# LeCAR-Lab/CoVO-MPC

Hardware: AMD Instinct MI355X
Metric: mpc_control_steps_per_sec (higher is better)
Workload: dtype f32; 1 GPU; covo-online tracking_zigzag N=65536 H=32 lam=0.01 sigma=0.5 (teacher-forced on the recorded inputs -- noisy state, a_mean, key -- of this controller's own 300-step closed-loop episode, timed steps spread evenly over the episode; samples sharded 1x65536, one exchange of the 516-float rank records per step: collective); controller=covo-online, task=tracking_zigzag, N_global=65536, N_local=65536, H=32, pos_stats_info=False

## Files before the change

covo_mpc_amd/csrc/hessian_adj_body.hpp:

```cpp
constexpr int NX = ADJ_NX, NZ = NX + 4, NH = NX + 1, HH = COVO_H, NA = COVO_NA;
constexpr size_t WS_X = 0;
constexpr size_t WS_JF = WS_X + 32 * 16;
constexpr size_t WS_GL = WS_JF + 32 * NX * NZ;
constexpr size_t WS_LAM = WS_GL + 32 * 16;
constexpr size_t WS_MXX = WS_LAM + 33 * 16;
constexpr size_t WS_MXU = WS_MXX + 32 * 256;
constexpr size_t WS_MUU = WS_MXU + 32 * 64;
constexpr size_t WS_S = WS_MUU + 32 * 16;
constexpr int NPAIR = NZ * (NZ + 1) / 2;
constexpr int PAIR_THREADS = (NPAIR + 63) / 64 * 64;
constexpr size_t WS_COUNT = WS_S + (size_t)32 * 16 * NA + 2;
constexpr unsigned long long ADJ_LAM_UNSET = 0xFFF7ADEADBEEF000ull;


__device__ __forceinline__ void adj_force(const float *__restrict__ st, const AdjArgs &A, int bi, int k, double (&f)[3])
{
    if (k == 0) {
        f[0] = st[ST_FDIST + 0]; f[1] = st[ST_FDIST + 1]; f[2] = st[ST_FDIST + 2];
    } else if (A.f_tab != nullptr) {
        const float4 r = A.f_tab[(size_t)bi * HH + k];
        f[0] = r.x; f[1] = r.y; f[2] = r.z;
    } else {
        f[0] = f[1] = f[2] = 0.0;
    }
}

__device__ __forceinline__ void adj_targets(const float *__restrict__ st, const float *__restrict__ pos_traj,
                                            const float *__restrict__ vel_traj, int T, int time0, int k, double (&tar)[6])
{
    if (k == 0) {
        for (int i = 0; i < 3; ++i) { tar[i] = st[ST_POSTAR + i]; tar[3 + i] = st[ST_VELTAR + i]; }
    } else {
        int idx = time0 + k;
        idx = idx < 0 ? 0 : (idx > T - 1 ? T - 1 : idx);
        for (int i = 0; i < 3; ++i) { tar[i] = pos_traj[3 * idx + i]; tar[3 + i] = vel_traj[3 * idx + i]; }
    }
}

#define ADJ_FOR_STATE(OP) OP(px, 0) OP(py, 1) OP(pz, 2) OP(vx, 3) OP(vy, 4) OP(vz, 5) OP(qx, 6) OP(qy, 7) OP(qz, 8) OP(qw, 9) OP(ox, 10) OP(oy, 11) OP(oz, 12)

__device__ __forceinline__ void adj_store_state(const qm::State<double> &p, double *__restrict__ x)
{
#define OP(m, i) x[i] = p.m;
    ADJ_FOR_STATE(OP)
#undef OP
}
__device__ __forceinline__ void adj_load_state(qm::State<double> &p, const double *__restrict__ x)
{
#define OP(m, i) p.m = x[i];
    ADJ_FOR_STATE(OP)
#undef OP
}

#if ADJ_FS
struct AdjDrag {
    double k, off[3];
};
__device__ __forceinline__ AdjDrag adj_drag(const AdjArgs &A, int bi)
{
    AdjDrag D = {A.drag_k, {A.drag_off[0], A.drag_off[1], A.drag_off[2]}};
    if (A.models != nullptr) {
        const dm::Model m = A.models[bi];
        D.k = adj_drag_coeff(m);
        for (int i = 0; i < 3; ++i) D.off[i] = 0.5 * (double)m.dp[i];
    }
    return D;
}
template <class S>
__device__ __forceinline__ void adj_next_force(const AdjArgs &A, const AdjDrag &D, int bi, int k, const qm::State<S> &s, const S (&f)[3],
                                               S (&fn)[3])
{
    if (k + 1 >= HH) {
        fn[0] = fn[1] = fn[2] = S{};
        return;
    }
    const float4 r = A.f_tab[(size_t)bi * HH + k + 1];
    const double g[3] = {r.x, r.y, r.z}, c = r.w;
    const S v[3] = {s.vx, s.vy, s.vz};
#pragma unroll
    for (int i = 0; i < 3; ++i) fn[i] = (f[i] * c + g[i]) + qm::drag_force<S, double>(v[i], D.off[i], D.k);
}
#endif


#if !ADJ_FS
struct AdjQuat {
    double x, y, z, w;
};
__device__ __forceinline__ AdjQuat adj_qmul(const AdjQuat &a, const AdjQuat &b)
{
    AdjQuat r;
    r.x = fma(a.w, b.x, fma(a.x, b.w, fma(a.y, b.z, -(a.z * b.y))));
    r.y = fma(a.w, b.y, fma(a.y, b.w, fma(a.z, b.x, -(a.x * b.z))));
    r.z = fma(a.w, b.z, fma(a.z, b.w, fma(a.x, b.y, -(a.y * b.x))));
    r.w = fma(a.w, b.w, -fma(a.x, b.x, fma(a.y, b.y, a.z * b.z)));
    return r;
}
template <int CTRL>
__device__ __forceinline__ AdjQuat adj_qdpp(const AdjQuat &q)
{
    return AdjQuat{wr::dpp_f64<CTRL>(q.x), wr::dpp_f64<CTRL>(q.y), wr::dpp_f64<CTRL>(q.z), wr::dpp_f64<CTRL>(q.w)};
}
__device__ __forceinline__ double adj_scan_sum(double v, const double (&pw)[4], double pr, int lane)
{
    v = fma(wr::dpp_f64<0x111>(v), pw[0], v);
    v = fma(wr::dpp_f64<0x112>(v), pw[1], v);
    v = fma(wr::dpp_f64<0x114>(v), pw[2], v);
    v = fma(wr::dpp_f64<0x118>(v), pw[3], v);
    const double t = wr::dpp_f64<0x142>(v);
    return ((lane & 16) != 0) ? fma(t, pr, v) : v;
}
template <bool FT>
__device__ __forceinline__ qm::State<double> adj_prefix_scan(const qm::State<double> &p0, const double (*sact)[4], const double (*sfd)[3],
                                                             const qm::Consts<double> &c, int lane)
{
    const int k = lane & 31, lo = lane & 15;
    const double one[4] = {1.0, 1.0, 1.0, 1.0};
    double pa[4];
    pa[0] = c.alpha;
    pa[1] = pa[0] * pa[0];
    pa[2] = pa[1] * pa[1];
    pa[3] = pa[2] * pa[2];
    const double a16 = pa[3] * pa[3];
    double alo = 1.0;
    if (lo & 1) alo *= pa[0];
    if (lo & 2) alo *= pa[1];
    if (lo & 4) alo *= pa[2];
    if (lo & 8) alo *= pa[3];
    const double ak = (k & 16) ? alo * a16 : alo, apr = alo * c.alpha;
    const double th = sact[k][0];
    double cx = sact[k][1] * c.one_m_alpha, cy = sact[k][2] * c.one_m_alpha, cz = sact[k][3] * c.one_m_alpha;
    cx = adj_scan_sum(cx, pa, apr, lane);
    cy = adj_scan_sum(cy, pa, apr, lane);
    cz = adj_scan_sum(cz, pa, apr, lane);
    const double ox = fma(ak, p0.ox, wr::dpp_f64<0x138>(cx));
    const double oy = fma(ak, p0.oy, wr::dpp_f64<0x138>(cy));
    const double oz = fma(ak, p0.oz, wr::dpp_f64<0x138>(cz));
    AdjQuat P{ox * c.half_dt, oy * c.half_dt, oz * c.half_dt, 1.0};
    {
        AdjQuat t = adj_qdpp<0x111>(P);
        if (lo >= 1) P = adj_qmul(t, P);
        t = adj_qdpp<0x112>(P);
        if (lo >= 2) P = adj_qmul(t, P);
        t = adj_qdpp<0x114>(P);
        if (lo >= 4) P = adj_qmul(t, P);
        t = adj_qdpp<0x118>(P);
        if (lo >= 8) P = adj_qmul(t, P);
        t = adj_qdpp<0x142>(P);
        if (lane & 16) P = adj_qmul(t, P);
    }
    AdjQuat E = adj_qdpp<0x138>(P);
    if (lane == 0) E = AdjQuat{0.0, 0.0, 0.0, 1.0};
    AdjQuat q0{p0.qx, p0.qy, p0.qz, p0.qw};
    {
        const double rn = qm::rsq64_(fma(q0.x, q0.x, fma(q0.y, q0.y, fma(q0.z, q0.z, q0.w * q0.w))));
        q0.x *= rn; q0.y *= rn; q0.z *= rn; q0.w *= rn;
    }
    AdjQuat q = adj_qmul(q0, E);
    if (k > 0) {
        const double rn = qm::rsq64_(fma(q.x, q.x, fma(q.y, q.y, fma(q.z, q.z, q.w * q.w))));
        q.x *= rn; q.y *= rn; q.z *= rn; q.w *= rn;
    }
    const double fx = (FT || k == 0) ? sfd[k][0] : 0.0, fy = (FT || k == 0) ? sfd[k][1] : 0.0, fz = (FT || k == 0) ? sfd[k][2] : 0.0;
    const double Qz0 = 2.0 * (q.x * q.z + q.y * q.w), Qz1 = 2.0 * (q.y * q.z - q.x * q.w), Qz2 = q.w * q.w - q.x * q.x - q.y * q.y + q.z * q.z;
    double dvx = ((Qz0 * th + fx) * c.inv_m) * c.dt, dvy = ((Qz1 * th + fy) * c.inv_m) * c.dt, dvz = ((Qz2 * th + fz) * c.inv_m + c.neg_g) * c.dt;
    dvx = adj_scan_sum(dvx, one, 1.0, lane);
    dvy = adj_scan_sum(dvy, one, 1.0, lane);
    dvz = adj_scan_sum(dvz, one, 1.0, lane);
    const double vx = p0.vx + wr::dpp_f64<0x138>(dvx), vy = p0.vy + wr::dpp_f64<0x138>(dvy), vz = p0.vz + wr::dpp_f64<0x138>(dvz);
    double dpx = adj_scan_sum(vx * c.dt, one, 1.0, lane), dpy = adj_scan_sum(vy * c.dt, one, 1.0, lane), dpz = adj_scan_sum(vz * c.dt, one, 1.0, lane);
    qm::State<double> r;
    r.px = p0.px + wr::dpp_f64<0x138>(dpx);
    r.py = p0.py + wr::dpp_f64<0x138>(dpy);
    r.pz = p0.pz + wr::dpp_f64<0x138>(dpz);
    r.vx = vx; r.vy = vy; r.vz = vz;
    r.qx = (k == 0) ? p0.qx : q.x; r.qy = (k == 0) ? p0.qy : q.y; r.qz = (k == 0) ? p0.qz : q.z; r.qw = (k == 0) ? p0.qw : q.w;
    r.ox = ox; r.oy = oy; r.oz = oz;
    return r;
}
#endif

__device__ __forceinline__ void adj_hd_step(const float *__restrict__ st, const float *__restrict__ am, const AdjArgs &A, int bi,
                                            int time0, int k, const qm::State<double> &p, int a, int b, qm::HD &r,
                                            qm::State<qm::HD> &s
#if ADJ_FS
                                            , const double (&pf)[3], qm::HD (&fn)[3]
#endif
)
{
    const qm::Consts<double> c = A.cs ? A.cs[bi] : A.c;
#define OP(m, i) s.m = qm::HD{p.m, a == i ? 1.0 : 0.0, b == i ? 1.0 : 0.0, 0.0};
    ADJ_FOR_STATE(OP)
#undef OP
#if ADJ_FS
    qm::HD fh[3];
#pragma unroll
    for (int i = 0; i < 3; ++i) {
        fh[i] = qm::HD{pf[i], a == 13 + i ? 1.0 : 0.0, b == 13 + i ? 1.0 : 0.0, 0.0};
        fn[i] = fh[i];
    }
#endif
    r = qm::hd(0.0);
    if (k >= 1) {
        double tar[6];
        adj_targets(st, A.pos_traj + bi * A.traj_stride, A.vel_traj + bi * A.traj_stride, A.T, time0, k, tar);
        r = qm::reward_kind<qm::HD, double>(A.reward, s, tar[0], tar[1], tar[2], tar[3], tar[4], tar[5]);
    }
    if (k <= HH - 2) {
        qm::HD act[4];
#pragma unroll
        for (int d = 0; d < 4; ++d) {
            const qm::HD x{(double)am[4 * k + d], a == NX + d ? 1.0 : 0.0, b == NX + d ? 1.0 : 0.0, 0.0};
            act[d] = qm::clip11_(qm::clip11_(x));
        }
#if ADJ_FS
        adj_next_force<qm::HD>(A, adj_drag(A, bi), bi, k, s, fh, fn);
        qm::dyn_step<qm::HD, double, true, qm::HD>(s, act[0], act[1], act[2], act[3], c, fh[0], fh[1], fh[2]);
#else
        double f[3];
        adj_force(st, A, bi, k, f);
        qm::dyn_step<qm::HD, double>(s, act[0], act[1], act[2], act[3], c, f[0], f[1], f[2]);
#endif
    }
}

template <bool FT>
__global__ __launch_bounds__(64) void adj_jac_kernel(const AdjArgs A)
{
    const int k = blockIdx.x, b = blockIdx.y, lane = threadIdx.x;
    const float *__restrict__ st = A.state + (size_t)b * COVO_STATE_FLOATS;
    const bool raw = A.a_mean_raw != nullptr;
    const float *__restrict__ am_base = raw ? A.a_mean_raw : A.a_mean + (size_t)b * NA;
    const bool shift = raw && A.begin_pass == 0;
    auto am = [&](int i) { return am_base[(shift && i < NA - 4) ? i + 4 : i]; };
    if (raw && k == 0) {
        float *shift_out = const_cast<float *>(A.a_mean);
        shift_out[lane] = am(lane);
        shift_out[lane + 64] = am(lane + 64);
        if (lane < 4) {
            if (A.begin_pass > 0) {
                const uint32_t p0 = A.dyn_out[10], p1 = A.dyn_out[11];
                uint32_t rk[2];
                step_begin_derive_next(lane, p0, p1, A.shared_noise_scale, A.dyn_out, rk);
            } else {
                step_begin_derive(lane, A.blk, A.derive_keys, A.shared_noise_scale, A.dyn_out);
            }
        }
        if (lane == 4 && A.seq != nullptr) A.seq[0] = A.seq[0] + 1u;
    }
    double *__restrict__ ws = A.ws + (size_t)b * WS_COUNT;
    if (lane < 16) {
        reinterpret_cast<unsigned long long *>(ws + WS_LAM)[16 * k + lane] = ADJ_LAM_UNSET;
        if (k == HH - 1) reinterpret_cast<unsigned long long *>(ws + WS_LAM)[16 * HH + lane] = ADJ_LAM_UNSET;
    }
    const int time0 = __float_as_int(st[ST_TIME]);
    const qm::Consts<double> c = A.cs ? A.cs[b] : A.c;
    qm::State<double> p;
    p.px = st[ST_POS + 0]; p.py = st[ST_POS + 1]; p.pz = st[ST_POS + 2];
    p.vx = st[ST_VEL + 0]; p.vy = st[ST_VEL + 1]; p.vz = st[ST_VEL + 2];
    p.qx = st[ST_QUAT + 0]; p.qy = st[ST_QUAT + 1]; p.qz = st[ST_QUAT + 2]; p.qw = st[ST_QUAT + 3];
    p.ox = st[ST_OMEGA + 0]; p.oy = st[ST_OMEGA + 1]; p.oz = st[ST_OMEGA + 2];
    __shared__ double sact[HH][4];
    __shared__ double sfd[HH][3];
    if (lane < HH) {
        double f[3];
        adj_force(st, A, b, lane, f);
        sfd[lane][0] = f[0]; sfd[lane][1] = f[1]; sfd[lane][2] = f[2];
    }
    if (lane < HH) {
        const double a0 = qm::clip11_((double)am(4 * lane + 0)), a1 = qm::clip11_((double)am(4 * lane + 1));
        const double a2 = qm::clip11_((double)am(4 * lane + 2)), a3 = qm::clip11_((double)am(4 * lane + 3));
        sact[lane][0] = (a0 + 1.0) * c.thrust_half;
        sact[lane][1] = a1 * c.komega[0];
        sact[lane][2] = a2 * c.komega[1];
        sact[lane][3] = a3 * c.komega[2];
    }
    __syncthreads();
#if ADJ_FS
    const AdjDrag D = adj_drag(A, b);
    double pf[3] = {sfd[0][0], sfd[0][1], sfd[0][2]};
    for (int t = 0; t < k; ++t) {
        const double th = sact[t][0], w0 = sact[t][1], w1 = sact[t][2], w2 = sact[t][3];
        double fn[3];
        adj_next_force<double>(A, D, b, t, p, pf, fn);
        if (t == 0) qm::dyn_core<double, double>(p, th, w0, w1, w2, c, pf[0], pf[1], pf[2]);
        else qm::dyn_core<double, double, false>(p, th, w0, w1, w2, c, pf[0], pf[1], pf[2]);
        pf[0] = fn[0]; pf[1] = fn[1]; pf[2] = fn[2];
    }
    if (lane == 0) {
        adj_store_state(p, ws + WS_X + 16 * k);
        ws[WS_X + 16 * k + 13] = pf[0]; ws[WS_X + 16 * k + 14] = pf[1]; ws[WS_X + 16 * k + 15] = pf[2];
    }
#else
    if (A.scan_prefix) {
        const qm::State<double> ps = adj_prefix_scan<FT>(p, sact, sfd, c, lane);
#define OP(m, i) p.m = wr::bcast_lane(ps.m, k);
        ADJ_FOR_STATE(OP)
#undef OP
    } else {
        for (int t = 0; t < k; ++t) {
            const double th = sact[t][0], w0 = sact[t][1], w1 = sact[t][2], w2 = sact[t][3];
            if (t == 0) qm::dyn_core<double, double>(p, th, w0, w1, w2, c, sfd[0][0], sfd[0][1], sfd[0][2]);
            else if (FT) qm::dyn_core<double, double, false>(p, th, w0, w1, w2, c, sfd[t][0], sfd[t][1], sfd[t][2]);
            else qm::dyn_core<double, double, false>(p, th, w0, w1, w2, c, 0.0, 0.0, 0.0);
        }
    }
    if (lane == 0) adj_store_state(p, ws + WS_X + 16 * k);
#endif
    qm::State<qm::D1> s;
#define OP(m, i) s.m = qm::D1{p.m, lane == i ? 1.0 : 0.0};
    ADJ_FOR_STATE(OP)
#undef OP
#if ADJ_FS
    qm::D1 fd[3], fdn[3];
#pragma unroll
    for (int i = 0; i < 3; ++i) {
        fd[i] = qm::D1{pf[i], lane == 13 + i ? 1.0 : 0.0};
        fdn[i] = fd[i];
    }
#endif
    qm::D1 r{0.0, 0.0};
    if (k >= 1) {
        double tar[6];
        adj_targets(st, A.pos_traj + b * A.traj_stride, A.vel_traj + b * A.traj_stride, A.T, time0, k, tar);
        r = qm::reward_kind<qm::D1, double>(A.reward, s, tar[0], tar[1], tar[2], tar[3], tar[4], tar[5]);
    }
    if (k <= HH - 2) {
        qm::D1 act[4];
#pragma unroll
        for (int d = 0; d < 4; ++d) {
            const qm::D1 x{(double)am(4 * k + d), lane == NX + d ? 1.0 : 0.0};
            act[d] = qm::clip11_(qm::clip11_(x));
        }
#if ADJ_FS
        adj_next_force<qm::D1>(A, D, b, k, s, fd, fdn);
        qm::dyn_step<qm::D1, double, true, qm::D1>(s, act[0], act[1], act[2], act[3], c, fd[0], fd[1], fd[2]);
#else
        qm::dyn_step<qm::D1, double>(s, act[0], act[1], act[2], act[3], c, sfd[k][0], sfd[k][1], sfd[k][2]);
#endif
    }
    if (lane < NZ) {
        if (lane < NX) ws[WS_GL + 16 * k + lane] = r.a;
        if (k <= HH - 2) {
            double *__restrict__ jf = ws + WS_JF + (size_t)k * NX * NZ;
#define OP(m, i) jf[i * NZ + lane] = s.m.a;
            ADJ_FOR_STATE(OP)
#undef OP
#if ADJ_FS
            jf[13 * NZ + lane] = fdn[0].a; jf[14 * NZ + lane] = fdn[1].a; jf[15 * NZ + lane] = fdn[2].a;
#endif
        }
    }
}

__device__ __forceinline__ void adj_hd_pairs(const AdjArgs &A, int k, int b, int tid)
{
    if (tid >= NPAIR) return;
    const float *__restrict__ st = A.state + (size_t)b * COVO_STATE_FLOATS;
    const float *__restrict__ am = A.a_mean + (size_t)b * NA;
    double *__restrict__ ws = A.ws + (size_t)b * WS_COUNT;
    const int time0 = __float_as_int(st[ST_TIME]);
    int q = tid, a = 0;
    while (q >= NZ - a) { q -= NZ - a; ++a; }
    const int bb = a + q;
    qm::State<double> p;
    adj_load_state(p, ws + WS_X + 16 * k);
    qm::HD r;
    qm::State<qm::HD> s;
#if ADJ_FS
    const double pf[3] = {ws[WS_X + 16 * k + 13], ws[WS_X + 16 * k + 14], ws[WS_X + 16 * k + 15]};
    qm::HD fn[3];
    adj_hd_step(st, am, A, b, time0, k, p, a, bb, r, s, pf, fn);
#else
    adj_hd_step(st, am, A, b, time0, k, p, a, bb, r, s);
#endif
    double h[NH];
    h[0] = r.ab;
#define OP(m, i) h[1 + i] = s.m.ab;
    ADJ_FOR_STATE(OP)
#undef OP
#if ADJ_FS
    h[14] = fn[0].ab; h[15] = fn[1].ab; h[16] = fn[2].ab;
#endif
    double g = h[0];
    if (k <= HH - 2) {
        const double *__restrict__ Lk = ws + WS_LAM + 16 * (k + 1);
        double lam[NX];
        const long long t0 = wall_clock64();
        for (;;) {
            bool unset = false;
#pragma unroll
            for (int i = 0; i < NX; ++i) {
                lam[i] = __hip_atomic_load(Lk + i, __ATOMIC_RELAXED, __HIP_MEMORY_SCOPE_AGENT);
                unset |= (unsigned long long)__double_as_longlong(lam[i]) == ADJ_LAM_UNSET;
            }
            if (!unset) break;
            if (wall_clock64() - t0 > 50000000LL) {
                if (A.status != nullptr) __hip_atomic_fetch_or(A.status, COVO_DEVSTAT_ADJOINT, __ATOMIC_RELAXED, __HIP_MEMORY_SCOPE_SYSTEM);
                break;
            }
            __builtin_amdgcn_s_sleep(2);
        }
#pragma unroll
        for (int i = 0; i < NX; ++i) g = fma(lam[i], h[1 + i], g);
    }
    double *__restrict__ Mxx = ws + WS_MXX + (size_t)k * 256, *__restrict__ Mxu = ws + WS_MXU + (size_t)k * 64;
    double *__restrict__ Muu = ws + WS_MUU + (size_t)k * 16;
    if (bb < NX) {
        Mxx[a * 16 + bb] = g;
        Mxx[bb * 16 + a] = g;
    } else if (a < NX) {
        Mxu[a * 4 + (bb - NX)] = g;
    } else {
        Muu[(a - NX) * 4 + (bb - NX)] = g;
        Muu[(bb - NX) * 4 + (a - NX)] = g;
    }
}

__device__ __forceinline__ void adj_hd_padding(const AdjArgs &A, int k, int b, int tid, int nthreads)
{
    double *__restrict__ ws = A.ws + (size_t)b * WS_COUNT;
    double *__restrict__ Mxx = ws + WS_MXX + (size_t)k * 256, *__restrict__ Mxu = ws + WS_MXU + (size_t)k * 64;
    for (int e = tid; e < 256; e += nthreads)
        if ((e >> 4) >= NX || (e & 15) >= NX) Mxx[e] = 0.0;
    if (tid < (16 - NX) * 4) Mxu[NX * 4 + tid] = 0.0;
}

__global__ __launch_bounds__(256) void adj_hd_kernel(const AdjArgs A)
{
    adj_hd_padding(A, (int)blockIdx.x, (int)blockIdx.y, (int)threadIdx.x, 256);
    adj_hd_pairs(A, (int)blockIdx.x, (int)blockIdx.y, (int)threadIdx.x);
}

static_assert(HH == 32, "adj_chain_kernel: four horizon segments of 8, 8, 8 and 7 steps");
constexpr int KC_ZI = (HH - 1) * NX * NZ;
constexpr int KC_TLD = 17;

__device__ __forceinline__ void adj_wave_sync()
{
    __builtin_amdgcn_fence(__ATOMIC_ACQ_REL, "wavefront");
    __builtin_amdgcn_wave_barrier();
}
__device__ __forceinline__ void adj_cd_to_a(double *__restrict__ tb, const f64x4 &t, int lo, int hi, double (&a)[4])
{
    adj_wave_sync();
#pragma unroll
    for (int r = 0; r < 4; ++r) tb[(4 * r + hi) * KC_TLD + lo] = t[r];
    adj_wave_sync();
#pragma unroll
    for (int g = 0; g < 4; ++g) a[g] = tb[lo * KC_TLD + 4 * g + hi];
}
__device__ __forceinline__ f64x4 adj_mm(const double (&a)[4], const f64x4 &b, f64x4 acc)
{
#pragma unroll
    for (int g = 0; g < 4; ++g) acc = __builtin_amdgcn_mfma_f64_16x16x4f64(a[g], b[g], acc, 0, 0, 0);
    return acc;
}
template <int CNT>
__device__ __forceinline__ void adj_mm_many(const double (&pa)[8][4], const f64x4 &b, f64x4 (&out)[8])
{
#pragma unroll
    for (int i = 0; i < CNT; ++i) out[i] = f64x4{0.0, 0.0, 0.0, 0.0};
#pragma unroll
    for (int g = 0; g < 4; ++g) {
#pragma unroll
        for (int i = 0; i < CNT; ++i) out[i] = __builtin_amdgcn_mfma_f64_16x16x4f64(pa[i][g], b[g], out[i], 0, 0, 0);
    }
}

template <int J>
__device__ __forceinline__ void adj_sens_chain(const double *__restrict__ sjf, double *__restrict__ tb, double *__restrict__ ho,
                                               double *__restrict__ S, int w, int lane, double (&pa)[8][4], f64x4 &sv)
{
    constexpr int M0 = 8 * J, M1 = J == 3 ? HH - 1 : 8 * J + 8;
    const int lo = lane & 15, hi = lane >> 4;
    const int col = 16 * w + lo, tcol = col >> 2, dcol = col & 3, k0 = 4 * w, jw = w >> 1;
    double *__restrict__ Sp = S + (size_t)hi * NA + col;
#pragma unroll
    for (int k = (J == 0 ? 0 : M0 + 1); k <= M1; ++k) {
        if (k <= k0) {
#pragma unroll
            for (int r = 0; r < 4; ++r) Sp[((size_t)k * 16 + 4 * r) * NA] = 0.0;
        }
    }
    if (J < jw) return;
    int offA[4];
    bool okA[4];
#pragma unroll
    for (int g = 0; g < 4; ++g) {
        okA[g] = lo < NX && 4 * g + hi < NX;
        offA[g] = lo * NZ + 4 * g + hi;
    }
    double an[4];
    if (J == jw) {
        sv = f64x4{0.0, 0.0, 0.0, 0.0};
        f64x4 bn;
#pragma unroll
        for (int g = 0; g < 4; ++g) an[g] = sjf[okA[g] ? k0 * NX * NZ + offA[g] : KC_ZI];
#pragma unroll
        for (int r = 0; r < 4; ++r) bn[r] = (tcol == k0 && hi + 4 * r < NX) ? sjf[(k0 * NX + hi + 4 * r) * NZ + NX + dcol] : 0.0;
#pragma unroll
        for (int k = M0; k < M1; ++k) {
            if (k < k0) continue;
            double ac[4];
            f64x4 acc = bn;
#pragma unroll
            for (int g = 0; g < 4; ++g) ac[g] = an[g];
            if (k + 1 < M1) {
#pragma unroll
                for (int g = 0; g < 4; ++g) an[g] = sjf[okA[g] ? (k + 1) * NX * NZ + offA[g] : KC_ZI];
                if (k + 1 <= k0 + 3) {
#pragma unroll
                    for (int r = 0; r < 4; ++r)
                        bn[r] = (tcol == k + 1 && hi + 4 * r < NX) ? sjf[((k + 1) * NX + hi + 4 * r) * NZ + NX + dcol] : 0.0;
                } else {
#pragma unroll
                    for (int r = 0; r < 4; ++r) bn[r] = 0.0;
                }
            }
            sv = adj_mm(ac, sv, acc);
#pragma unroll
            for (int r = 0; r < 4; ++r) Sp[((size_t)(k + 1) * 16 + 4 * r) * NA] = sv[r];
        }
        if (J < 3) {
#pragma unroll
            for (int r = 0; r < 4; ++r) ho[64 * r + lane] = sv[r];
        }
    } else if constexpr (J > 0) {
        f64x4 t;
#pragma unroll
        for (int r = 0; r < 4; ++r) t[r] = sjf[(lo < NX && 4 * r + hi < NX) ? M0 * NX * NZ + (4 * r + hi) * NZ + lo : KC_ZI];
#pragma unroll
        for (int g = 0; g < 4; ++g) pa[0][g] = sjf[okA[g] ? M0 * NX * NZ + offA[g] : KC_ZI];
#pragma unroll
        for (int g = 0; g < 4; ++g) an[g] = sjf[okA[g] ? (M0 + 1) * NX * NZ + offA[g] : KC_ZI];
#pragma unroll
        for (int k = M0 + 1; k < M1; ++k) {
            double ac[4];
#pragma unroll
            for (int g = 0; g < 4; ++g) ac[g] = an[g];
            if (k + 1 < M1) {
#pragma unroll
                for (int g = 0; g < 4; ++g) an[g] = sjf[okA[g] ? (k + 1) * NX * NZ + offA[g] : KC_ZI];
            }
            t = adj_mm(ac, t, f64x4{0.0, 0.0, 0.0, 0.0});
            adj_cd_to_a(tb, t, lo, hi, pa[k - M0]);
        }
    }
}
template <int J>
__device__ __forceinline__ void adj_sens_join(const double *__restrict__ hi_slot, double *__restrict__ ho, int lane,
                                              const double (&pa)[8][4], f64x4 &sm, f64x4 &sv)
{
    constexpr int CNT = J == 3 ? HH - 1 - 24 : 8;
#pragma unroll
    for (int r = 0; r < 4; ++r) sm[r] = hi_slot[64 * r + lane];
    sv = adj_mm(pa[CNT - 1], sm, f64x4{0.0, 0.0, 0.0, 0.0});
    if (J < 3) {
#pragma unroll
        for (int r = 0; r < 4; ++r) ho[64 * r + lane] = sv[r];
    }
}
template <int J>
__device__ __forceinline__ void adj_sens_fill(double *__restrict__ S, int w, int lane, const double (&pa)[8][4], const f64x4 &sm,
                                              const f64x4 &sv)
{
    constexpr int M0 = 8 * J, M1 = J == 3 ? HH - 1 : 8 * J + 8, CNT = M1 - M0;
    double *__restrict__ Sp = S + (size_t)(lane >> 4) * NA + 16 * w + (lane & 15);
#pragma unroll
    for (int r = 0; r < 4; ++r) Sp[((size_t)M1 * 16 + 4 * r) * NA] = sv[r];
    f64x4 out[8];
    adj_mm_many<CNT - 1>(pa, sm, out);
#pragma unroll
    for (int i = 0; i < CNT - 1; ++i) {
#pragma unroll
        for (int r = 0; r < 4; ++r) Sp[((size_t)(M0 + 1 + i) * 16 + 4 * r) * NA] = out[i][r];
    }
}

template <int KEND>
__device__ __forceinline__ void adj_cost_top(const double *__restrict__ sjf, const double *__restrict__ G, double *__restrict__ L,
                                             int lane, f64x4 &lam)
{
    const int lo = lane & 15, hi = lane >> 4;
#pragma unroll
    for (int r = 0; r < 4; ++r) lam[r] = (lo == 0 && hi + 4 * r < NX) ? G[16 * (HH - 1) + hi + 4 * r] : 0.0;
    if (lo == 0) {
#pragma unroll
        for (int r = 0; r < 4; ++r) {
            __hip_atomic_store(&L[16 * (HH - 1) + hi + 4 * r], lam[r], __ATOMIC_RELAXED, __HIP_MEMORY_SCOPE_AGENT);
            __hip_atomic_store(&L[16 * HH + hi + 4 * r], 0.0, __ATOMIC_RELAXED, __HIP_MEMORY_SCOPE_AGENT);
        }
    }
    int offA[4];
    bool okA[4];
#pragma unroll
    for (int g = 0; g < 4; ++g) {
        okA[g] = lo < NX && 4 * g + hi < NX;
        offA[g] = (4 * g + hi) * NZ + lo;
    }
    bool okG[4];
#pragma unroll
    for (int r = 0; r < 4; ++r) okG[r] = lo == 0 && hi + 4 * r < NX;
    double an[4];
    f64x4 gn;
#pragma unroll
    for (int g = 0; g < 4; ++g) an[g] = sjf[okA[g] ? (HH - 2) * NX * NZ + offA[g] : KC_ZI];
#pragma unroll
    for (int r = 0; r < 4; ++r) gn[r] = okG[r] ? G[16 * (HH - 2) + hi + 4 * r] : 0.0;
#pragma unroll
    for (int k = HH - 2; k >= KEND; --k) {
        double ac[4];
        f64x4 acc = gn;
#pragma unroll
        for (int g = 0; g < 4; ++g) ac[g] = an[g];
        if (k > KEND) {
#pragma unroll
            for (int g = 0; g < 4; ++g) an[g] = sjf[okA[g] ? (k - 1) * NX * NZ + offA[g] : KC_ZI];
#pragma unroll
            for (int r = 0; r < 4; ++r) gn[r] = okG[r] ? G[16 * (k - 1) + hi + 4 * r] : 0.0;
        }
        lam = adj_mm(ac, lam, acc);
        if (lo == 0) {
#pragma unroll
            for (int r = 0; r < 4; ++r) __hip_atomic_store(&L[16 * k + hi + 4 * r], lam[r], __ATOMIC_RELAXED, __HIP_MEMORY_SCOPE_AGENT);
        }
    }
}
#if !ADJ_FS
template <int J>
__device__ __forceinline__ void adj_cost_chain(const double *__restrict__ sjf, const double *__restrict__ G, double *__restrict__ tb,
                                               int lane, double (&pa)[8][4])
{
    constexpr int E = 8 * J + 7, M = J == 0 ? 1 : 8 * J;
    const int lo = lane & 15, hi = lane >> 4;
    int offA[4], offT[4];
    bool okA[4], okG[4];
#pragma unroll
    for (int g = 0; g < 4; ++g) {
        okA[g] = lo < NX && 4 * g + hi < NX;
        offA[g] = (4 * g + hi) * NZ + lo;
        offT[g] = lo * NZ + 4 * g + hi;
        okG[g] = lo == NX && 4 * g + hi < NX;
    }
    f64x4 t;
#pragma unroll
    for (int r = 0; r < 4; ++r) {
        const double a = sjf[okA[r] ? E * NX * NZ + offT[r] : KC_ZI];
        t[r] = okG[r] ? G[16 * E + hi + 4 * r] : a;
    }
#pragma unroll
    for (int g = 0; g < 4; ++g) {
        const double a = sjf[okA[g] ? E * NX * NZ + offA[g] : KC_ZI];
        pa[0][g] = (4 * g + hi == NX && lo < NX) ? G[16 * E + lo] : a;
    }
    double an[4];
    f64x4 gn;
#pragma unroll
    for (int g = 0; g < 4; ++g) an[g] = sjf[okA[g] ? (E - 1) * NX * NZ + offA[g] : KC_ZI];
#pragma unroll
    for (int r = 0; r < 4; ++r) gn[r] = okG[r] ? G[16 * (E - 1) + hi + 4 * r] : 0.0;
#pragma unroll
    for (int k = E - 1; k >= M; --k) {
        double ac[4];
        f64x4 acc = gn;
#pragma unroll
        for (int g = 0; g < 4; ++g) ac[g] = an[g];
        if (k > M) {
#pragma unroll
            for (int g = 0; g < 4; ++g) an[g] = sjf[okA[g] ? (k - 1) * NX * NZ + offA[g] : KC_ZI];
#pragma unroll
            for (int r = 0; r < 4; ++r) gn[r] = okG[r] ? G[16 * (k - 1) + hi + 4 * r] : 0.0;
        }
        t = adj_mm(ac, t, acc);
        adj_cd_to_a(tb, t, lo, hi, pa[E - k]);
    }
}
__device__ __forceinline__ double adj_cost_quarter(const double (&a)[4], const double (&vv)[4])
{
    return fma(a[3], vv[3], fma(a[2], vv[2], fma(a[1], vv[1], a[0] * vv[0])));
}
__device__ __forceinline__ double adj_cost_over_hi(double p)
{
    p += __shfl_xor(p, 16, 64);
    p += __shfl_xor(p, 32, 64);
    return p;
}
__device__ __forceinline__ void adj_cost_publish(double *__restrict__ L, int k, int lane, double v)
{
    if (lane < 16) __hip_atomic_store(&L[16 * k + lane], v, __ATOMIC_RELAXED, __HIP_MEMORY_SCOPE_AGENT);
}
__device__ __forceinline__ void adj_flag_set(int *flag)
{
    adj_wave_sync();
    __hip_atomic_store(flag, 1, __ATOMIC_RELEASE, __HIP_MEMORY_SCOPE_WORKGROUP);
}
__device__ __forceinline__ void adj_flag_wait(int *flag, const AdjArgs &A)
{
    const long long t0 = wall_clock64();
    while (__hip_atomic_load(flag, __ATOMIC_ACQUIRE, __HIP_MEMORY_SCOPE_WORKGROUP) == 0) {
        if (wall_clock64() - t0 > 50000000LL) {
            if (A.status != nullptr) __hip_atomic_fetch_or(A.status, COVO_DEVSTAT_ADJOINT, __ATOMIC_RELAXED, __HIP_MEMORY_SCOPE_SYSTEM);
            break;
        }
        __builtin_amdgcn_s_sleep(1);
    }
}
template <int J>
__device__ __forceinline__ void adj_cost_join(const double *__restrict__ hi_slot, double *__restrict__ ho, int *flag,
                                              double *__restrict__ L, int lane, const double (&pa)[8][4], double (&vv)[4])
{
    constexpr int E = 8 * J + 7, M = J == 0 ? 1 : 8 * J;
    const int hi = lane >> 4;
#pragma unroll
    for (int g = 0; g < 4; ++g) {
        const double x = hi_slot[4 * g + hi];
        vv[g] = 4 * g + hi < NX ? x : (4 * g + hi == NX ? 1.0 : 0.0);
    }
    const double lm = adj_cost_over_hi(adj_cost_quarter(pa[E - M], vv));
    if (J > 0) {
        if (lane < 16) ho[lane] = lm;
        adj_flag_set(flag);
    }
    adj_cost_publish(L, M, lane, lm);
}
template <int J>
__device__ __forceinline__ void adj_cost_fill(double *__restrict__ L, int lane, const double (&pa)[8][4], const double (&vv)[4])
{
    constexpr int E = 8 * J + 7, M = J == 0 ? 1 : 8 * J;
    double q[E - M];
#pragma unroll
    for (int i = 0; i < E - M; ++i) q[i] = adj_cost_quarter(pa[i], vv);
#pragma unroll
    for (int i = 0; i < E - M; ++i) q[i] += __shfl_xor(q[i], 16, 64);
#pragma unroll
    for (int i = 0; i < E - M; ++i) q[i] += __shfl_xor(q[i], 32, 64);
#pragma unroll
    for (int i = 0; i < E - M; ++i) adj_cost_publish(L, E - i, lane, q[i]);
}
#endif

__global__ __launch_bounds__(256) void adj_chain_kernel(const AdjArgs A)
{
    __shared__ double sjf[(HH - 1) * NX * NZ + 1];
    __shared__ double sgl[HH * 16];
    __shared__ double stb[4][16 * KC_TLD];
    __shared__ double sho[3][256];
    __shared__ int sfl[4];
    const int b = blockIdx.y, tid = threadIdx.x, lane = tid & 63, wv = tid >> 6;
    const int w = blockIdx.x;
    double *__restrict__ ws = A.ws + (size_t)b * WS_COUNT;
#ifdef KC_STAMPS
    const long long kc0 = wall_clock64();
    long long kc3 = 0, kc4 = 0;
#define KC_STAMP(x) x = (long long)wall_clock64() - kc0
#else
#define KC_STAMP(x) do { } while (0)
#endif
    if (w >= 9) {
        adj_hd_padding(A, w - 9, b, tid, 256);
        adj_hd_pairs(A, w - 9, b, tid);
#ifdef KC_STAMPS
        if (tid == 0 && b == 0 && ((w - 9) % 8 == 0 || w - 9 == HH - 1)) printf("KC hd %d: end %lld (10 ns ticks from entry)\n", w - 9, (long long)wall_clock64() - kc0);
#endif
        return;
    }
    {
        constexpr int NJ = (HH - 1) * NX * NZ, TJ = (NJ + 255) / 256;
        double vj[TJ];
#pragma unroll
        for (int t = 0; t < TJ; ++t) vj[t] = (tid + 256 * t < NJ) ? ws[WS_JF + tid + 256 * t] : 0.0;
        const double vg0 = ws[WS_GL + tid], vg1 = ws[WS_GL + 256 + tid];
#pragma unroll
        for (int t = 0; t < TJ; ++t)
            if (tid + 256 * t < NJ) sjf[tid + 256 * t] = vj[t];
        sgl[tid] = vg0;
        sgl[256 + tid] = vg1;
        if (tid == 0) sjf[NJ] = 0.0;
        if (tid < 4) sfl[tid] = 0;
    }
#ifdef KC_STAMPS
    const long long kc1 = wall_clock64();
#endif
    __syncthreads();
#ifdef KC_STAMPS
    const long long kc2 = wall_clock64();
    __shared__ long long kcs[4][4];
#define KC_STAMP_END(ALL)                                                                                                    \
    do {                                                                                                                     \
        const long long kc5 = (long long)wall_clock64() - kc0;                                                               \
        asm volatile("s_waitcnt vmcnt(0)" ::: "memory");                                                                     \
        if (lane == 0) { kcs[wv][0] = kc3; kcs[wv][1] = kc4; kcs[wv][2] = kc5; kcs[wv][3] = (long long)wall_clock64() - kc0; } \
        if (ALL) __syncthreads();                                                                                            \
        if (tid == 0 && b == 0 && (w == 0 || w == 7 || w == 8))                                                              \
            for (int q = 0; q < (ALL ? 4 : 1); ++q)                                                                          \
                printf("KC wg %d wave %d: filled %lld first-mfma %lld segment %lld join %lld end %lld acked %lld (10 ns "    \
                       "ticks from entry)\n", w, q, kc1 - kc0, kc2 - kc0, kcs[q][0], kcs[q][1], kcs[q][2], kcs[q][3]);       \
    } while (0)
#else
#define KC_STAMP_END(ALL) do { } while (0)
#endif
    double pa[8][4];
    if (w == 8) {
        double *__restrict__ L = ws + WS_LAM;
        f64x4 lam;
#if ADJ_FS
        if (wv != 0) return;
        adj_cost_top<1>(sjf, sgl, L, lane, lam);
        KC_STAMP(kc3);
#else
        double vv[4];
        switch (wv) {
        case 0:
            adj_cost_chain<0>(sjf, sgl, stb[0], lane, pa);
            KC_STAMP(kc3);
            adj_flag_wait(&sfl[2], A);
            adj_cost_join<0>(sho[2], sho[2], &sfl[2], L, lane, pa, vv);
            KC_STAMP(kc4);
            adj_cost_fill<0>(L, lane, pa, vv);
            break;
        case 1:
            adj_cost_chain<1>(sjf, sgl, stb[1], lane, pa);
            KC_STAMP(kc3);
            adj_flag_wait(&sfl[1], A);
            adj_cost_join<1>(sho[1], sho[2], &sfl[2], L, lane, pa, vv);
            KC_STAMP(kc4);
            adj_cost_fill<1>(L, lane, pa, vv);
            break;
        case 2:
            adj_cost_chain<2>(sjf, sgl, stb[2], lane, pa);
            KC_STAMP(kc3);
            adj_flag_wait(&sfl[0], A);
            adj_cost_join<2>(sho[0], sho[1], &sfl[1], L, lane, pa, vv);
            KC_STAMP(kc4);
            adj_cost_fill<2>(L, lane, pa, vv);
            break;
        default:
            adj_cost_top<24>(sjf, sgl, L, lane, lam);
            if ((lane & 15) == 0) {
#pragma unroll
                for (int r = 0; r < 4; ++r) sho[0][(lane >> 4) + 4 * r] = lam[r];
            }
            adj_flag_set(&sfl[0]);
            KC_STAMP(kc3);
        }
#endif
        KC_STAMP_END(!ADJ_FS);
        return;
    }
    double *__restrict__ S = ws + WS_S;
    const int jw = w >> 1;
    f64x4 sv, sm;
    switch (wv) {
    case 0: adj_sens_chain<0>(sjf, stb[0], sho[0], S, w, lane, pa, sv); break;
    case 1: adj_sens_chain<1>(sjf, stb[1], sho[1], S, w, lane, pa, sv); break;
    case 2: adj_sens_chain<2>(sjf, stb[2], sho[2], S, w, lane, pa, sv); break;
    default: adj_sens_chain<3>(sjf, stb[3], sho[2], S, w, lane, pa, sv);
    }
    KC_STAMP(kc3);
    __syncthreads();
    if (wv == 1 && jw < 1) { adj_sens_join<1>(sho[0], sho[1], lane, pa, sm, sv); KC_STAMP(kc4); }
    __syncthreads();
    if (wv == 2 && jw < 2) { adj_sens_join<2>(sho[1], sho[2], lane, pa, sm, sv); KC_STAMP(kc4); }
    __syncthreads();
    if (wv == 3 && jw < 3) { adj_sens_join<3>(sho[2], sho[2], lane, pa, sm, sv); KC_STAMP(kc4); }
    if (wv > jw) {
        if (wv == 1) adj_sens_fill<1>(S, w, lane, pa, sm, sv);
        else if (wv == 2) adj_sens_fill<2>(S, w, lane, pa, sm, sv);
        else adj_sens_fill<3>(S, w, lane, pa, sm, sv);
    }
    KC_STAMP_END(true);
}
#undef KC_STAMP_END
#undef KC_STAMP

__device__ __forceinline__ void adj_tri_tile(int w, int &ti, int &tj)
{
    ti = 0;
    while ((ti + 1) * (ti + 2) / 2 <= w) ++ti;
    tj = w - ti * (ti + 1) / 2;
}

__global__ __launch_bounds__(512) void adj_gemm_kernel(const AdjArgs A)
{
    __shared__ double red[8][4][64];
    __shared__ double sMu[4][64];
    __shared__ double sMuu[64];
    const int b = blockIdx.y, tid = threadIdx.x, lane = tid & 63, wv = tid >> 6, lo = lane & 15, hi = lane >> 4;
    const double *__restrict__ ws = A.ws + (size_t)b * WS_COUNT;
    double *__restrict__ R = A.R + (size_t)b * NA * NA;
    int I, J;
    adj_tri_tile(blockIdx.x, I, J);
    const double *__restrict__ S = ws + WS_S, *__restrict__ Mxx = ws + WS_MXX;
    f64x4 acc = {0.0, 0.0, 0.0, 0.0};
#ifdef KD_PROF
    const long long kp0 = clock64();
#endif
    double ma[4][4], sj[4][4], si[4][4];
#pragma unroll
    for (int it = 0; it < 4; ++it) {
        const int k = 4 * I + 1 + wv + 8 * it;
        const bool on = k < HH;
        const double *__restrict__ Sk = S + (size_t)(on ? k : 0) * 16 * NA, *__restrict__ Mk = Mxx + (size_t)(on ? k : 0) * 256;
        const double2 *__restrict__ Mk2 = reinterpret_cast<const double2 *>(Mk + lo * 16 + 4 * hi);
        const double2 m01 = on ? Mk2[0] : make_double2(0.0, 0.0), m23 = on ? Mk2[1] : make_double2(0.0, 0.0);
        ma[it][0] = m01.x;
        ma[it][1] = m01.y;
        ma[it][2] = m23.x;
        ma[it][3] = m23.y;
#pragma unroll
        for (int g = 0; g < 4; ++g) {
            sj[it][g] = on ? Sk[(size_t)(4 * hi + g) * NA + 16 * J + lo] : 0.0;
            si[it][g] = on ? Sk[(size_t)(4 * g + hi) * NA + 16 * I + lo] : 0.0;
        }
    }
    const int i = 16 * I + hi + 4 * (wv & 3), j = 16 * J + lo;
    const int ti = i >> 2, di = i & 3, tj = j >> 2, dj = j & 3;
    const int tk = ti > tj ? ti : tj, dk = ti > tj ? di : dj;
    double es[NX];
    if (wv < 4) {
        const int col = ti > tj ? j : i;
        const double *__restrict__ Sk = S + (size_t)tk * 16 * NA;
#pragma unroll
        for (int m = 0; m < NX; ++m) es[m] = Sk[(size_t)m * NA + col];
    } else if (wv == 4) {
        sMuu[lane] = ws[WS_MUU + (size_t)(4 * I) * 16 + lane];
    }
    if (tid < 256) sMu[wv][lane] = ws[WS_MXU + (size_t)(4 * I + wv) * 64 + lane];
    __shared__ double sNan;
    const double lz = (wv == 5 && lane < 16) ? ws[WS_LAM + 16 + lane] : 0.0;
#ifdef KD_PROF
    asm volatile("s_waitcnt vmcnt(0)" ::: "memory");
    const long long kp1 = clock64();
#endif
#pragma unroll
    for (int it = 0; it < 4; ++it) {
        if (4 * I + 1 + wv + 8 * it >= HH) break;
        f64x4 Q = {0.0, 0.0, 0.0, 0.0};
#pragma unroll
        for (int g = 0; g < 4; ++g) Q = __builtin_amdgcn_mfma_f64_16x16x4f64(ma[it][g], sj[it][g], Q, 0, 0, 0);
#pragma unroll
        for (int g = 0; g < 4; ++g) acc = __builtin_amdgcn_mfma_f64_16x16x4f64(si[it][g], Q[g], acc, 0, 0, 0);
    }
    if (wv == 5) {
        double pz = lz * 0.0;
        pz += __shfl_xor(pz, 1, 64);
        pz += __shfl_xor(pz, 2, 64);
        pz += __shfl_xor(pz, 4, 64);
        pz += __shfl_xor(pz, 8, 64);
        if (lane == 0) sNan = pz;
    }
#pragma unroll
    for (int r = 0; r < 4; ++r) red[wv][r][lane] = acc[r];
#ifdef KD_PROF
    const long long kp2 = clock64();
#endif
    __syncthreads();
#ifdef KD_PROF
    const long long kp3 = clock64();
    if (tid == 0 && (blockIdx.x == 0 || blockIdx.x == 35)) printf("KD wg %d: loads %lld mfma %lld barrier %lld\n", (int)blockIdx.x, kp1 - kp0, kp2 - kp1, kp3 - kp2);
#endif
    double v = 0.0;
    if (wv < 4) {
#pragma unroll
        for (int w8 = 0; w8 < 8; ++w8) v += red[w8][wv][lane];
        if (ti != tj) {
            const double *mu = sMu[tk - 4 * I];
#pragma unroll
            for (int m = 0; m < NX; ++m) v = fma(es[m], mu[m * 4 + dk], v);
        } else {
            v += sMuu[(ti - 4 * I) * 16 + di * 4 + dj];
        }
        const double pz = sNan;
        if (pz != pz) v = pz;
        if (I != J || i >= j) {
            R[(size_t)i * NA + j] = -v;
            R[(size_t)j * NA + i] = -v;
        }
    }
    if (A.stats.rpart != nullptr) {
        __shared__ double st_tmp[16][17];
        __shared__ double st_part[4];
        __shared__ double st_diag[16][17];
        double rv = -v;
        if (I == J) {
            if (wv < 4) st_diag[hi + 4 * wv][lo] = rv;
            __syncthreads();
            if (wv < 4 && i < j) rv = st_diag[lo][hi + 4 * wv];
        }
        SymStatsOut so = A.stats;
        so.rpart += (size_t)b * so.stride;
        so.fpart += (size_t)b * so.stride;
        so.diag += (size_t)b * so.stride;
        sym_tile_stats(wv < 4, rv, I, J, (int)blockIdx.x, lane, wv & 3, so, st_tmp, st_part);
        if (so.flags != nullptr && blockIdx.x == 0 && tid < 64) so.flags[(size_t)b * so.stride + tid] = 0.0;
        if (so.ready != nullptr && blockIdx.x == 0 && tid == 64) so.ready[(size_t)b * so.stride] = 0.0;
    }
}
#undef ADJ_FOR_STATE
```

Before: 6371 control-steps/s.

## Specialize adj GEMM waves by live k-count and reuse sj via permlane transpose on diagonal

Replaces the fixed four-iteration load/MFMA loop, which masked inactive k with zeros, with a templated per-wave path that is dispatched on the number of live k slices, the diagonal-tile case and whether the wave needs the epilogue es loads. Idle waves no longer issue dead loads or MFMAs. On diagonal tiles the si operand comes from a permlane32/permlane16 register transpose of sj instead of a second global load. The epilogue scalar loads are merged into a single per-wave pointer and issued alongside the main loads, with sched_barriers to order load issue ahead of the MFMAs. This adds a wide switch of template instantiations, which grows code size and may change register pressure.

New measurement: 6382 control-steps/s, median of 3. Within noise of the previous version (+0.2%).

```diff
diff --git a/covo_mpc_amd/csrc/hessian_adj_body.hpp b/covo_mpc_amd/csrc/hessian_adj_body.hpp
--- a/covo_mpc_amd/csrc/hessian_adj_body.hpp
+++ b/covo_mpc_amd/csrc/hessian_adj_body.hpp
@@ -881,6 +881,75 @@
     tj = w - ti * (ti + 1) / 2;
 }
 
+__device__ __forceinline__ void adj_rows_regs_transpose(const double (&x)[4], double (&y)[4])
+{
+    unsigned w[4][2], p[4][2];
+#pragma unroll
+    for (int g = 0; g < 4; ++g) {
+        w[g][0] = (unsigned)__double2loint(x[g]);
+        w[g][1] = (unsigned)__double2hiint(x[g]);
+    }
+#pragma unroll
+    for (int h = 0; h < 2; ++h) {
+#pragma unroll
+        for (int g = 0; g < 2; ++g) {
+            const auto r = __builtin_amdgcn_permlane32_swap(w[g][h], w[g + 2][h], false, false);
+            p[g][h] = r[0];
+            p[g + 2][h] = r[1];
+        }
+#pragma unroll
+        for (int g = 0; g < 4; g += 2) {
+            const auto r = __builtin_amdgcn_permlane16_swap(p[g][h], p[g + 1][h], false, false);
+            w[g][h] = r[0];
+            w[g + 1][h] = r[1];
+        }
+    }
+#pragma unroll
+    for (int g = 0; g < 4; ++g) y[g] = __hiloint2double((int)w[g][1], (int)w[g][0]);
+}
+
+template <int NL, bool FIN, bool DIAG>
+__device__ __forceinline__ void adj_gemm_wave(const double *__restrict__ S, const double *__restrict__ Mxx, const double *__restrict__ esp,
+                                              const double *__restrict__ evp, int I, int J, int wv, int lo, int hi, f64x4 &acc,
+                                              double (&es)[NX], double &ev)
+{
+    double ma[NL > 0 ? NL : 1][4], sj[NL > 0 ? NL : 1][4], si[NL > 0 ? NL : 1][4];
+#pragma unroll
+    for (int it = 0; it < NL; ++it) {
+        const int k = 4 * I + 1 + wv + 8 * it;
+        const double *__restrict__ Sk = S + (size_t)k * 16 * NA, *__restrict__ Mk = Mxx + (size_t)k * 256;
+        const double2 *__restrict__ Mk2 = reinterpret_cast<const double2 *>(Mk + lo * 16 + 4 * hi);
+        const double2 m01 = Mk2[0], m23 = Mk2[1];
+        ma[it][0] = m01.x;
+        ma[it][1] = m01.y;
+        ma[it][2] = m23.x;
+        ma[it][3] = m23.y;
+#pragma unroll
+        for (int g = 0; g < 4; ++g) sj[it][g] = Sk[(size_t)(4 * hi + g) * NA + 16 * J + lo];
+        if (!DIAG) {
+#pragma unroll
+            for (int g = 0; g < 4; ++g) si[it][g] = Sk[(size_t)(4 * g + hi) * NA + 16 * I + lo];
+        }
+        __builtin_amdgcn_sched_barrier(0);
+    }
+    if (FIN) {
+#pragma unroll
+        for (int m = 0; m < NX; ++m) es[m] = esp[(size_t)m * NA];
+    }
+    ev = *evp;
+    __builtin_amdgcn_sched_barrier(0);
+#pragma unroll
+    for (int it = 0; it < NL; ++it) {
+        f64x4 Q = {0.0, 0.0, 0.0, 0.0};
+#pragma unroll
+        for (int g = 0; g < 4; ++g) Q = __builtin_amdgcn_mfma_f64_16x16x4f64(ma[it][g], sj[it][g], Q, 0, 0, 0);
+        if (DIAG) adj_rows_regs_transpose(sj[it], si[it]);
+#pragma unroll
+        for (int g = 0; g < 4; ++g) acc = __builtin_amdgcn_mfma_f64_16x16x4f64(si[it][g], Q[g], acc, 0, 0, 0);
+        __builtin_amdgcn_sched_barrier(0);
+    }
+}
+
 __global__ __launch_bounds__(512) void adj_gemm_kernel(const AdjArgs A)
 {
     __shared__ double red[8][4][64];
@@ -896,54 +965,41 @@
 #ifdef KD_PROF
     const long long kp0 = clock64();
 #endif
-    double ma[4][4], sj[4][4], si[4][4];
-#pragma unroll
-    for (int it = 0; it < 4; ++it) {
-        const int k = 4 * I + 1 + wv + 8 * it;
-        const bool on = k < HH;
-        const double *__restrict__ Sk = S + (size_t)(on ? k : 0) * 16 * NA, *__restrict__ Mk = Mxx + (size_t)(on ? k : 0) * 256;
-        const double2 *__restrict__ Mk2 = reinterpret_cast<const double2 *>(Mk + lo * 16 + 4 * hi);
-        const double2 m01 = on ? Mk2[0] : make_double2(0.0, 0.0), m23 = on ? Mk2[1] : make_double2(0.0, 0.0);
-        ma[it][0] = m01.x;
-        ma[it][1] = m01.y;
-        ma[it][2] = m23.x;
-        ma[it][3] = m23.y;
-#pragma unroll
-        for (int g = 0; g < 4; ++g) {
-            sj[it][g] = on ? Sk[(size_t)(4 * hi + g) * NA + 16 * J + lo] : 0.0;
-            si[it][g] = on ? Sk[(size_t)(4 * g + hi) * NA + 16 * I + lo] : 0.0;
-        }
-    }
     const int i = 16 * I + hi + 4 * (wv & 3), j = 16 * J + lo;
     const int ti = i >> 2, di = i & 3, tj = j >> 2, dj = j & 3;
     const int tk = ti > tj ? ti : tj, dk = ti > tj ? di : dj;
-    double es[NX];
-    if (wv < 4) {
-        const int col = ti > tj ? j : i;
-        const double *__restrict__ Sk = S + (size_t)tk * 16 * NA;
-#pragma unroll
-        for (int m = 0; m < NX; ++m) es[m] = Sk[(size_t)m * NA + col];
-    } else if (wv == 4) {
-        sMuu[lane] = ws[WS_MUU + (size_t)(4 * I) * 16 + lane];
-    }
-    if (tid < 256) sMu[wv][lane] = ws[WS_MXU + (size_t)(4 * I + wv) * 64 + lane];
     __shared__ double sNan;
-    const double lz = (wv == 5 && lane < 16) ? ws[WS_LAM + 16 + lane] : 0.0;
+    const int swv = __builtin_amdgcn_readfirstlane(wv);
+    const double *__restrict__ evp = swv < 4 ? ws + WS_MXU + (size_t)(4 * I + swv) * 64 + lane
+                                             : (swv == 4 ? ws + WS_MUU + (size_t)(4 * I) * 16 + lane : ws + WS_LAM + 16 + lo);
+    const double *__restrict__ esp = S + (size_t)tk * 16 * NA + (ti > tj ? j : i);
+    double es[NX], ev;
+    {
+        const int nl = (38 - 4 * I - swv) >> 3;
+#define KD_WAVE(N, D)                                                                                                \
+    case 4 * N + 2 * D: adj_gemm_wave<N, false, D != 0>(S, Mxx, esp, evp, I, J, swv, lo, hi, acc, es, ev); break;    \
+    case 4 * N + 2 * D + 1: adj_gemm_wave<N, true, D != 0>(S, Mxx, esp, evp, I, J, swv, lo, hi, acc, es, ev); break;
+        switch (4 * nl + (I == J ? 2 : 0) + (swv < 4 ? 1 : 0)) {
+            KD_WAVE(0, 0)
+            KD_WAVE(0, 1)
+            KD_WAVE(1, 0)
+            KD_WAVE(1, 1)
+            KD_WAVE(2, 0)
+            KD_WAVE(2, 1)
+            KD_WAVE(3, 0)
+            KD_WAVE(3, 1)
+            KD_WAVE(4, 0)
+            KD_WAVE(4, 1)
+        }
+#undef KD_WAVE
+    }
 #ifdef KD_PROF
-    asm volatile("s_waitcnt vmcnt(0)" ::: "memory");
     const long long kp1 = clock64();
 #endif
-#pragma unroll
-    for (int it = 0; it < 4; ++it) {
-        if (4 * I + 1 + wv + 8 * it >= HH) break;
-        f64x4 Q = {0.0, 0.0, 0.0, 0.0};
-#pragma unroll
-        for (int g = 0; g < 4; ++g) Q = __builtin_amdgcn_mfma_f64_16x16x4f64(ma[it][g], sj[it][g], Q, 0, 0, 0);
-#pragma unroll
-        for (int g = 0; g < 4; ++g) acc = __builtin_amdgcn_mfma_f64_16x16x4f64(si[it][g], Q[g], acc, 0, 0, 0);
-    }
-    if (wv == 5) {
-        double pz = lz * 0.0;
+    if (swv < 4) sMu[swv][lane] = ev;
+    else if (swv == 4) sMuu[lane] = ev;
+    else if (swv == 5) {
+        double pz = ev * 0.0;
         pz += __shfl_xor(pz, 1, 64);
         pz += __shfl_xor(pz, 2, 64);
         pz += __shfl_xor(pz, 4, 64);
@@ -958,7 +1014,7 @@
     __syncthreads();
 #ifdef KD_PROF
     const long long kp3 = clock64();
-    if (tid == 0 && (blockIdx.x == 0 || blockIdx.x == 35)) printf("KD wg %d: loads %lld mfma %lld barrier %lld\n", (int)blockIdx.x, kp1 - kp0, kp2 - kp1, kp3 - kp2);
+    if (tid == 0 && (blockIdx.x == 0 || blockIdx.x == 35)) printf("KD wg %d: entry to last MFMA %lld epilogue loads + LDS %lld barrier %lld\n", (int)blockIdx.x, kp1 - kp0, kp2 - kp1, kp3 - kp2);
 #endif
     double v = 0.0;
     if (wv < 4) {
```
